# mueller-franzes/medfusion

Measured on AMD Instinct MI355X. Metric: images/sec at 256x256, 150 DDIM steps (DiffusionPipeline.sample incl. VAE decode), higher is better.
Workload: dtype f32 (emulated: fp16 pairs -- 23-bit operands, and 23-bit STORAGE of the tensors between the UNet's conv blocks: they exist as fp16 pairs only)

## Files before the change

### medfusion_amd/csrc/conv_f16x2.h

```cpp
#pragma once
#include "common.h"
#include "split_f16.h"

#ifndef MFC2_HZ
#define MFC2_HZ 0
#endif
#ifndef MFC2_OUT_STORE
#define MFC2_OUT_STORE 0
#endif

namespace mfc2 {
using namespace mf;

typedef float f32x16 __attribute__((ext_vector_type(16)));
typedef float f32x4 __attribute__((ext_vector_type(4)));
typedef unsigned int u32x4 __attribute__((ext_vector_type(4)));
typedef _Float16 f16x8 __attribute__((ext_vector_type(8)));
typedef _Float16 f16x2 __attribute__((ext_vector_type(2)));

struct FuseP {
  int on, act;
  float eps, bconst;
  double count;
  const float* gamma;
  const float* beta;
  const float* res_f32;
  const void* res_pairs;
  const float* res_bound;
  const float* res_slots;
  int res_nslots;
  int tiles_per_sample;
  const float* emb;
  long emb_stride;
  const float* emb_bound;
  float* out_f32;
  void* out_pairs;
  float* out_bound;
  unsigned* rv;
  unsigned* rv_err;
};

struct ConvP2 {
  const void* x1;
  const void* x2;
  const void* w;
  const float* bias;
  float* y;
  const float* bound1;
  const float* bound2;
  int wexp;
  float* out_bound;
  int bound_slots;
  int N, Hin, Win, C1, C2, Cin, Cout;
  int Hout, Wout, Heff, Weff, KH, KW, stride, pad;
  int M, K, HWout;
  int cgroups, cg_per_split, splitk;
  int tiles_m, tiles_n;
  long slab;
  unsigned bytes1, bytes2, bytesw;
  int subpix, hw_src;
  int out_nt;
  int wphase_rows;
  int walk_n_fast;
  double* gn_partial;
  int gn_groups, gn_parts, gn_cpg;
  int tree;
  float* handoff;
  unsigned* sync;
  FuseP fz;
  void* y_pairs;
  float* y_pair_bound;
  float wl1_1, wl1_2, bmax;
#if MFC2_HZ & (256 | 512)
  float* dbg;
#endif
};

__device__ __forceinline__ int xcd_remap2(int bid, int total) {
  const int q = total >> 3, r = total & 7;
  const int xcd = bid & 7, within = bid >> 3;
  const int base = xcd < r ? xcd * (q + 1) : r * (q + 1) + (xcd - r) * q;
  return base + within;
}

#ifndef MFC2_HZ
#define MFC2_HZ 0
#endif
#define MFC2_HZ_ON(BIT) ((MFC2_HZ >> (BIT)) & 1)
#ifndef MFC2_HZ_PAD
#define MFC2_HZ_PAD 7
#endif

__device__ __forceinline__ float hz_add(float a, float b) { float r; asm volatile("v_add_f32 %0, %1, %2" : "=v"(r) : "v"(a), "v"(b)); return r; }
__device__ __forceinline__ float hz_mul(float a, float b) { float r; asm volatile("v_mul_f32 %0, %1, %2" : "=v"(r) : "v"(a), "v"(b)); return r; }

#define MFC2_WAIT_VM(N) asm volatile("s_waitcnt vmcnt(%0)" ::"n"(N) : "memory")
#if MFC2_HZ & 512
#define MFC2_STAMP(I) { if (p.dbg && threadIdx.x == 0) reinterpret_cast<unsigned long*>(p.dbg)[(long)MFC2_BID * 8 + (I)] = __builtin_amdgcn_s_memrealtime(); }
#else
#define MFC2_STAMP(I)
#endif
#define MFC2_WAIT_LGKM0() asm volatile("s_waitcnt lgkmcnt(0)" ::: "memory")

#define MFC2_BODY_AS_KERNEL 1
#define MFC2_BID blockIdx.x
#include "conv_f16x2_body.inc"
#undef MFC2_BODY_AS_KERNEL
#undef MFC2_BID
#define MFC2_BODY_AS_KERNEL 0
#define MFC2_BID bid
#include "conv_f16x2_body.inc"
#undef MFC2_BODY_AS_KERNEL
#undef MFC2_BID

__global__ __launch_bounds__(256) void split_act_f16x2_kernel(const float* __restrict__ x, u32x4* __restrict__ out, long octets,
                                                              const float* __restrict__ bound, long octets_per_row) {
  const long stride = (long)gridDim.x * blockDim.x;
  for (long o = (long)blockIdx.x * blockDim.x + threadIdx.x; o < octets; o += stride) {
    const float sc = bound ? exp2i(-scale_exp_of(bound[o / octets_per_row])) : 1.f;
    const f32x4 v0 = *reinterpret_cast<const f32x4*>(x + o * 8) * sc, v1 = *reinterpret_cast<const f32x4*>(x + o * 8 + 4) * sc;
    u32x4 hi, lo;
    split8_f16(v0, v1, hi, lo);
    out[o * 2] = hi;
    out[o * 2 + 1] = lo;
  }
}

__global__ __launch_bounds__(256) void split_act_slots_kernel(const float* __restrict__ x, u32x4* __restrict__ out, long octets_per_row,
                                                              const float* __restrict__ slots, int nslots, float* __restrict__ bound_out) {
  __shared__ float sm[4];
  const int row = blockIdx.y, tid = threadIdx.x;
  float m = 0.f;
  for (int i = tid; i < nslots; i += 256) m = fmaxf(m, slots[(long)row * nslots + i]);
  m = mf::wave_max(m);
  if ((tid & 63) == 0) sm[tid >> 6] = m;
  __syncthreads();
  const float b = fmaxf(fmaxf(sm[0], sm[1]), fmaxf(sm[2], sm[3]));
  if (blockIdx.x == 0 && tid == 0) bound_out[row] = b;
  const float sc = exp2i(-scale_exp_of(b));
  const long base = (long)row * octets_per_row;
  for (long o = (long)blockIdx.x * 256 + tid; o < octets_per_row; o += (long)gridDim.x * 256) {
    const f32x4 v0 = *reinterpret_cast<const f32x4*>(x + (base + o) * 8) * sc, v1 = *reinterpret_cast<const f32x4*>(x + (base + o) * 8 + 4) * sc;
    u32x4 hi, lo;
    split8_f16(v0, v1, hi, lo);
    out[(base + o) * 2] = hi;
    out[(base + o) * 2 + 1] = lo;
  }
}

}
```

### medfusion_amd/csrc/conv_f16x2.hip

```cpp
#include "common.h"
#include <string.h>
#include <mutex>
#include <vector>
#include "gn_partial.h"
#include "conv_plan.h"
#include "conv_f16x2.h"
#include "conv_f16x2_halo.h"
#include "conv_f16x2_group.h"
#include "winograd.h"

using namespace mf;

namespace {

struct Tile2 { int id, BM, BN, WM, WN, NST, HG; };
const Tile2 kTiles2[] = {
    {31, 128, 256, 2, 4, 3, 0}, {32, 256, 128, 4, 2, 3, 0}, {33, 128, 128, 2, 4, 3, 0}, {34, 128, 128, 4, 2, 3, 0}, {35, 256, 64, 4, 2, 3, 0},
    {36, 128, 64, 4, 2, 3, 0}, {37, 64, 256, 1, 8, 3, 0},
    {51, 128, 128, 2, 2, 2, 0}, {52, 128, 128, 2, 2, 3, 0}, {53, 64, 128, 2, 2, 3, 0}, {54, 128, 64, 2, 2, 3, 0},
    {61, 256, 128, 4, 2, 3, 6}, {62, 256, 128, 4, 2, 3, 7}, {63, 128, 128, 2, 4, 3, 4}, {64, 128, 128, 2, 4, 3, 5},
};
inline size_t tile_lds(const Tile2& t) {
  return t.HG ? (size_t)2 * t.HG * (t.WM * t.WN) * 1024 + (size_t)3 * t.BN * 128 : (size_t)t.NST * (t.BM + t.BN) * 128;
}
// ... 338 lines not shown
  return igemm_plan_query(d, tile_id, splitk);
}

int mf_split_f16x2(const float* x, void* xs, const float* bound, int rows, int64_t per_row, void* stream) {
  MF_REQUIRE(x && xs && rows > 0 && per_row > 0 && per_row % 8 == 0, MF_EINVAL, "split_f16x2: bad args (per_row %% 8 == 0)");
  const long octets = (long)rows * (per_row / 8);
  ProfScope ps(MF_FAM_MISC, (hipStream_t)stream, 0, 8.0 * rows * (double)per_row);
  const int blocks = (int)((octets + 255) / 256 > 8192 ? 8192 : (octets + 255) / 256);
  MF_LAUNCH(mfc2::split_act_f16x2_kernel, dim3(blocks), dim3(256), 0, (hipStream_t)stream, x, reinterpret_cast<mfc2::u32x4*>(xs), octets, bound,
                     (long)(per_row / 8));
  return check_launch("split_f16x2");
}

int mf_split_f16x2_slots(const float* x, void* xs, const float* slots, int nslots, float* bound_out, int rows, int64_t per_row, void* stream) {
  MF_REQUIRE(x && xs && slots && bound_out && nslots > 0 && rows > 0 && rows <= 65535 && per_row > 0 && per_row % 8 == 0, MF_EINVAL,
             "split_f16x2_slots: bad args (per_row %% 8 == 0, rows <= 65535)");
  const long opr = per_row / 8;
  ProfScope ps(MF_FAM_MISC, (hipStream_t)stream, 0, 8.0 * rows * (double)per_row);
  long bpr = (opr + 255) / 256;
  const long cap = (8192 + rows - 1) / rows;
  if (bpr > cap) bpr = cap;
  MF_LAUNCH(mfc2::split_act_slots_kernel, dim3((int)bpr, rows), dim3(256), 0, (hipStream_t)stream, x, reinterpret_cast<mfc2::u32x4*>(xs), opr, slots, nslots,
            bound_out);
  return check_launch("split_f16x2_slots");
}

static int host_scale_exp(float bound) {
  if (!(bound > 0.f)) return 0;
  uint32_t u;
  memcpy(&u, &bound, 4);
  const int s = (int)((u >> 23) & 0xffu) - 127 - 14;
  return s < -100 ? -100 : (s > 100 ? 100 : s);
}

int mf_conv2d_plan_override(const MfConvDesc* d, int tile, int splitk) {
  MF_REQUIRE(d && pair_precision(d->precision), MF_EINVAL, "plan_override: a MF_CONV_FP32_F16X2 / MF_CONV_F16 descriptor");
  std::lock_guard<std::mutex> lk(g_plan_mu);
  const int Cin = d->C1 + d->C2;
  for (size_t i = 0; i < g_plan_overrides.size(); ++i) {
    const PlanEntry& e = g_plan_overrides[i];
    if (e.N == d->N && e.H == d->Hin && e.W == d->Win && e.Cin == Cin && e.Cout == d->Cout && e.k == d->KH && e.stride == d->stride && e.ups == d->upsample) {
      g_plan_overrides.erase(g_plan_overrides.begin() + i);
      break;
    }
  }
  if (tile > 0 && splitk > 0) g_plan_overrides.push_back(PlanEntry{d->N, d->Hin, d->Win, Cin, d->Cout, d->KH, d->stride, d->upsample, tile, splitk});
  return MF_OK;
}

int mf_conv2d_f16x2_sync_words(const MfConvDesc* d) {
  Plan2 pl;
  if (!d || !pair_precision(d->precision) || make_plan2(d, &pl) != MF_OK || !pl.ok || !tree_possible(d, pl)) return 0;
  return cdiv(pl.M, pl.t.BM) * (d->Cout / pl.t.BN) * (pl.splitk - 1);
}

static int fuse_tiles_per_sample(const MfConvDesc* d, const Plan2& pl, int G) {
  if (!pl.ok || G <= 0 || G > 256 || d->Cout % G || d->upsample != 0) return 0;
  if (pl.splitk > 1 && !tree_possible(d, pl)) return 0;
  if (!epilogue_stats_ok(d, pl, G)) return 0;
  const int HW = pl.Hout * pl.Wout;
  if (HW < pl.t.BM && pl.t.BM / HW > 8) return 0;
  const long grid = (long)cdiv(pl.M, pl.t.BM) * (d->Cout / pl.t.BN) * pl.splitk;
  mfc2::ConvP2 dummy{};
  const int resident = dispatch_tile(pl.t.id, dummy, nullptr, d->precision == MF_CONV_F16 ? 1 : 3, 1);
  if (resident <= 0 || grid > resident) return 0;
  static const int fault = [] { const char* e = getenv("MEDFUSION_FUSE_FAULT"); return e ? atoi(e) : 0; }();
  return (HW >= pl.t.BM ? HW / pl.t.BM : 1) * (d->Cout / pl.t.BN) + (fault ? 1 : 0);
}

int mf_conv2d_f16x2_fuse_words(const MfConvDesc* d, int G) {
  Plan2 pl;
  if (!d || !pair_precision(d->precision) || make_plan2(d, &pl) != MF_OK || !pl.ok) return 0;
  return fuse_tiles_per_sample(d, pl, G) > 0 ? 2 * d->N : 0;
}

struct PairsOut { void* y_split; float* y_bound; float wl1_1, wl1_2, bmax; };
static int conv_f16x2_impl(const void* x1s, const void* x2s, const void* ws, const float* bias, float* y, const float* x1_bound, const float* x2_bound,
                           float w_bound, float* y_bound, void* workspace, size_t workspace_bytes, uint32_t* sync, double* gn_partial, int G,
                           const MfGnFuse* fz, const MfConvDesc* d, void* stream, const PairsOut* po = nullptr);

int mf_conv2d_f16x2_pairs_out_ok(const MfConvDesc* d) {
  Plan2 pl;
  if (!d || !pair_precision(d->precision) || make_plan2(d, &pl) != MF_OK || !pl.ok || d->Cout % 8) return 0;
  return (pl.splitk == 1 || tree_possible(d, pl)) ? 1 : 0;
}

int mf_conv2d_f16x2_pairs_out(const void* x1s, const void* x2s, const void* ws, const float* bias, float* y, void* y_split, float* y_bound_out,
                              const float* x1_bound, const float* x2_bound, float w_bound, float w_l1_1, float w_l1_2, float bias_max, void* workspace,
                              size_t workspace_bytes, uint32_t* sync, const MfConvDesc* d, void* stream) {
  MF_REQUIRE(y && y_split && y_bound_out && x1_bound, MF_EINVAL, "conv(f16x2, pairs out): y, y_split, y_bound_out and x1_bound are required");
  MF_REQUIRE(d && (d->C2 == 0 || x2_bound), MF_EINVAL, "conv(f16x2, pairs out): x2_bound with a second source");
  MF_REQUIRE(mf_conv2d_f16x2_pairs_out_ok(d), MF_EUNSUPPORTED, "conv(f16x2, pairs out): this plan reduces split-K behind the launch (mf_conv2d_f16x2_pairs_out_ok == 0)");
  MF_REQUIRE(w_l1_1 >= 0.f && w_l1_2 >= 0.f && bias_max >= 0.f, MF_EINVAL, "conv(f16x2, pairs out): norms must be >= 0");
  const PairsOut po{y_split, y_bound_out, w_l1_1, w_l1_2, bias_max};
  return conv_f16x2_impl(x1s, x2s, ws, bias, y, x1_bound, x2_bound, w_bound, nullptr, workspace, workspace_bytes, sync, nullptr, 0, nullptr, d, stream, &po);
}

int mf_conv2d_f16x2(const void* x1s, const void* x2s, const void* ws, const float* bias, float* y, const float* x1_bound, const float* x2_bound,
                    float w_bound, float* y_bound, void* workspace, size_t workspace_bytes, uint32_t* sync, double* gn_partial, int G,
                    const MfConvDesc* d, void* stream) {
  MF_REQUIRE(y, MF_EINVAL, "conv(f16x2): null pointer");
  return conv_f16x2_impl(x1s, x2s, ws, bias, y, x1_bound, x2_bound, w_bound, y_bound, workspace, workspace_bytes, sync, gn_partial, G, nullptr, d, stream);
}

int mf_conv2d_f16x2_gn_apply(const void* x1s, const void* x2s, const void* ws, const float* bias, const float* x1_bound, const float* x2_bound,
                             float w_bound, void* workspace, size_t workspace_bytes, uint32_t* sync, double* gn_partial, int G, const MfGnFuse* f,
                             const MfConvDesc* d, void* stream) {
  MF_REQUIRE(f && gn_partial && G > 0, MF_EINVAL, "conv_gn_apply: needs the fuse arguments, the record array and G");
  MF_REQUIRE(f->out_split && f->out_bound && f->rendezvous && f->error_flag, MF_EINVAL, "conv_gn_apply: out_split, out_bound, rendezvous and error_flag are required");
  MF_REQUIRE((f->gamma == nullptr) == (f->beta == nullptr), MF_EINVAL, "conv_gn_apply: gamma/beta must both be given or both NULL");
  MF_REQUIRE(!(f->residual && f->residual_pairs), MF_EINVAL, "conv_gn_apply: the residual is fp32 OR fp16 pairs");
  MF_REQUIRE(!f->residual_pairs || f->res_bound, MF_EINVAL, "conv_gn_apply: a residual given as fp16 pairs needs the res_bound that scaled it");
  MF_REQUIRE(!f->residual || f->res_bound || (f->res_bound_slots && f->res_nslots > 0), MF_EINVAL, "conv_gn_apply: a residual needs res_bound or res_bound_slots");
  MF_REQUIRE(!f->emb || (f->emb_bound && f->emb_stride % 4 == 0), MF_EINVAL, "conv_gn_apply: an embedding needs emb_bound and emb_stride %% 4 == 0");
  return conv_f16x2_impl(x1s, x2s, ws, bias, nullptr, x1_bound, x2_bound, w_bound, nullptr, workspace, workspace_bytes, sync, gn_partial, G, f, d, stream);
}

struct Prep { mfc2::ConvP2 p; Plan2 pl; bool tree; double flops, bytes; int terms; };
static int conv_f16x2_prepare(const void* x1s, const void* x2s, const void* ws, const float* bias, float* y, const float* x1_bound, const float* x2_bound,
                              float w_bound, float* y_bound, void* workspace, size_t workspace_bytes, uint32_t* sync, double* gn_partial, int G,
                              const MfGnFuse* fz, const MfConvDesc* d, const PairsOut* po, Prep* out, bool wino_gemm = false) {
  MF_REQUIRE(d && pair_precision(d->precision), MF_EINVAL, "conv(f16x2): desc.precision must be MF_CONV_FP32_F16X2 (or the opt-in MF_CONV_F16)");
  MF_REQUIRE((d->upsample == 3) == wino_gemm, MF_EINVAL, "conv(f16x2): upsample = 3 is internal to mf_conv2d_wino_f16x2");
  Plan2& pl = out->pl;
  mfc2::ConvP2& p = out->p;
  int rc = make_plan2(d, &pl);
  if (rc) return rc;
  MF_REQUIRE(pl.ok, MF_EUNSUPPORTED, "conv(f16x2): this shape/layout is not on the fp16-pair path (ask mf_conv2d_f16x2_ok)");
  MF_REQUIRE(x1s && ws && (y || fz), MF_EINVAL, "conv(f16x2): null pointer");
  MF_REQUIRE(d->C2 == 0 || x2s != nullptr, MF_EINVAL, "conv(f16x2): C2 > 0 but x2 is null");
  MF_REQUIRE(!gn_partial || gn_parts2(d, pl, G) > 0, MF_EUNSUPPORTED, "conv(f16x2): cannot emit GroupNorm partials (mf_conv2d_gn_parts == 0)");
  MF_REQUIRE(!y_bound || (!gn_partial && bound_slots2(d, pl, false) > 0), MF_EUNSUPPORTED,
             "conv(f16x2): cannot measure the output bound of this plan (mf_conv2d_f16x2_bound_slots == 0, or GroupNorm statistics requested)");
  p.x1 = x1s; p.x2 = x2s; p.w = ws; p.bias = bias; p.y = y;
  p.bound1 = x1_bound; p.bound2 = x2_bound; p.wexp = host_scale_exp(w_bound); p.out_bound = y_bound; p.bound_slots = y_bound ? bound_slots2(d, pl, false) : 0;
  p.N = d->N; p.Hin = d->Hin; p.Win = d->Win; p.C1 = d->C1; p.C2 = d->C2; p.Cin = d->C1 + d->C2; p.Cout = d->Cout;
  p.Hout = pl.Hout; p.Wout = pl.Wout; p.Heff = pl.Heff; p.Weff = pl.Weff;
  p.KH = d->KH; p.KW = d->KW; p.stride = d->stride; p.pad = d->pad;
  p.subpix = d->upsample == 2 ? 1 : 0; p.hw_src = d->Hin * d->Win;
  if (p.subpix) { p.KH = p.KW = 2; p.Heff = d->Hin; p.Weff = d->Win; }
  p.M = pl.M; p.K = pl.K; p.HWout = pl.Hout * pl.Wout;
  p.cgroups = pl.cgroups; p.cg_per_split = pl.cg_per_split; p.splitk = pl.splitk;
  p.tiles_m = cdiv(pl.M, pl.t.BM); p.tiles_n = d->Cout / pl.t.BN;
  p.slab = (long)pl.M * d->Cout;
  p.bytes1 = (unsigned)(4.0 * d->N * d->Hin * d->Win * d->C1);
  p.bytes2 = (unsigned)(4.0 * d->N * d->Hin * d->Win * d->C2);
  p.bytesw = (unsigned)(4.0 * d->Cout * pl.K * (p.subpix ? 4 : wino_gemm ? 16 : 1));
  p.wphase_rows = wino_gemm ? (d->N / 16) * d->Hin * d->Win : 0;
  {
    static const int walk = [] { const char* e = getenv("MF_CONV_WALK"); return e ? atoi(e) : 1; }();
    const double act_bytes = 4.0 * d->N * d->Hin * d->Win * (d->C1 + d->C2), w_bytes = 4.0 * d->Cout * pl.K * (p.subpix ? 4 : 1);
    p.walk_n_fast = (!wino_gemm && p.tiles_n > 1 && (walk == 2 || (walk == 1 && act_bytes > w_bytes))) ? 1 : 0;
  }
  p.out_nt = 0;
  p.gn_partial = nullptr; p.gn_groups = G; p.gn_cpg = G > 0 ? d->Cout / G : 8; p.gn_parts = 0;
  p.tree = 0; p.handoff = nullptr; p.sync = nullptr;
#if MFC2_HZ & (256 | 512)
  p.dbg = g_conv_dbg;
#endif
  p.y_pairs = po ? po->y_split : nullptr; p.y_pair_bound = po ? po->y_bound : nullptr;
  p.wl1_1 = po ? po->wl1_1 : 0.f; p.wl1_2 = po ? po->wl1_2 : 0.f; p.bmax = po ? po->bmax : 0.f;
  memset(&p.fz, 0, sizeof(p.fz));
  if (fz) {
    const int tps = fuse_tiles_per_sample(d, pl, G);
    MF_REQUIRE(tps > 0, MF_EUNSUPPORTED, "conv_gn_apply: this plan cannot apply its GroupNorm inside the launch (mf_conv2d_f16x2_fuse_words == 0)");
    p.fz.on = 1; p.fz.act = fz->act; p.fz.eps = fz->eps; p.fz.bconst = fz->bconst; p.fz.count = (double)(pl.Hout * pl.Wout) * (d->Cout / G);
    p.fz.gamma = fz->gamma; p.fz.beta = fz->beta; p.fz.res_f32 = fz->residual; p.fz.res_pairs = fz->residual_pairs;
    p.fz.res_bound = fz->res_bound; p.fz.res_slots = fz->res_bound ? nullptr : fz->res_bound_slots; p.fz.res_nslots = fz->res_nslots;
    p.fz.tiles_per_sample = tps; p.fz.emb = fz->emb; p.fz.emb_stride = (long)fz->emb_stride; p.fz.emb_bound = fz->emb_bound;
    p.fz.out_f32 = fz->out; p.fz.out_pairs = fz->out_split; p.fz.out_bound = fz->out_bound; p.fz.rv = fz->rendezvous; p.fz.rv_err = fz->error_flag;
  }
  const bool tree = pl.splitk > 1 && tree_possible(d, pl) && (!gn_partial || epilogue_stats_ok(d, pl, G));
  if ((pl.splitk == 1 || tree) && gn_partial) { p.gn_partial = gn_partial; p.gn_parts = p.HWout >= pl.t.BM ? p.HWout / pl.t.BM : 1; }
  if (tree) {
    const size_t need = tree_handoff_bytes(d, pl);
    MF_REQUIRE(workspace && workspace_bytes >= need, MF_EWORKSPACE, "conv(f16x2): workspace %zu < %zu", workspace_bytes, need);
    MF_REQUIRE(sync, MF_EINVAL, "conv(f16x2): this plan meets its split-K slices inside the launch and needs `sync` "
                                "(mf_conv2d_f16x2_sync_words(d) zero-initialised words the caller keeps between launches)");
    p.tree = tree_mode(); p.handoff = reinterpret_cast<float*>(workspace); p.sync = sync;
    if (y_bound && p.bound_slots == 0) p.out_bound = nullptr;
  } else if (pl.splitk > 1) {
    const size_t need = (size_t)pl.splitk * pl.M * d->Cout * sizeof(float);
    MF_REQUIRE(workspace && workspace_bytes >= need, MF_EWORKSPACE, "conv(f16x2): workspace %zu < %zu", workspace_bytes, need);
    p.y = reinterpret_cast<float*>(workspace);
    p.out_bound = nullptr;
  }
  out->tree = tree;
  out->flops = 2.0 * pl.M * (double)d->Cout * (d->upsample == 2 ? 9.0 * (d->C1 + d->C2) : (double)pl.K);
  out->bytes = 4.0 * ((double)d->N * d->Hin * d->Win * p.Cin + (double)d->Cout * pl.K + (double)pl.M * d->Cout);
  out->terms = d->precision == MF_CONV_F16 ? 1 : 3;
  return MF_OK;
}

static int conv_f16x2_impl(const void* x1s, const void* x2s, const void* ws, const float* bias, float* y, const float* x1_bound, const float* x2_bound,
                           float w_bound, float* y_bound, void* workspace, size_t workspace_bytes, uint32_t* sync, double* gn_partial, int G,
                           const MfGnFuse* fz, const MfConvDesc* d, void* stream, const PairsOut* po) {
  Prep q;
  int rc = conv_f16x2_prepare(x1s, x2s, ws, bias, y, x1_bound, x2_bound, w_bound, y_bound, workspace, workspace_bytes, sync, gn_partial, G, fz, d, po, &q);
  if (rc) return rc;
  hipStream_t s = (hipStream_t)stream;
  const Plan2& pl = q.pl;
  const mfc2::ConvP2& p = q.p;
  const bool tree = q.tree;
  {
    const int terms = q.terms;
    ProfScope ps(fz ? MF_FAM_CONV_GN_FUSED : MF_FAM_CONV_IGEMM, s, q.flops, q.bytes, 2.0 * pl.M * (double)d->Cout * pl.K * terms);
    ps.set_tag(pl.t.id + (terms == 1 ? 100000 : 0));
    rc = dispatch_tile(pl.t.id, p, s, terms, 0);
    if (rc == -1) { set_error("conv(f16x2): no tile config %d", pl.t.id); rc = MF_EINVAL; }
  }
  if (rc) return rc;
  if (pl.splitk > 1 && !tree) {
    const int HW = p.HWout;
    ProfScope ps(MF_FAM_SPLITK_REDUCE, s, 0, 4.0 * pl.M * d->Cout * (pl.splitk + 1));
    if (gn_partial) {
      const int slices = stats_slices(d->N, HW, d->Cout, G), chunks = stats_chunks(HW);
      MF_LAUNCH(gn_partial_kernel<true>, dim3(chunks, d->N, slices), dim3(kStatsThreads), stats_lds_bytes(d->Cout / slices), s,
                         reinterpret_cast<const float*>(workspace), gn_partial, HW, d->Cout, G, pl.splitk, p.slab, bias, y, (float*)nullptr);
      return check_launch("splitk_reduce_stats");
    }
    const long p4 = (long)HW * d->Cout / 4;
    int bx = (int)((p4 + 255) / 256);
    const int cap = cdiv(2048, d->N);
    if (bx > cap) bx = cap;
    MF_LAUNCH(splitk_reduce_kernel<0>, dim3(bx, d->N), dim3(256), 0, s, reinterpret_cast<const float*>(workspace), bias, y, p4, d->Cout,
                       pl.splitk, p.slab, y_bound);
    return check_launch("splitk_reduce");
  }
  return MF_OK;
}

static bool single_launch(const MfConvDesc* d, const Plan2& pl, int G) {
  if (pl.splitk == 1) return G == 0 || gn_parts2(d, pl, G) > 0;
  return tree_possible(d, pl) && (G == 0 || epilogue_stats_ok(d, pl, G));
}

int mf_conv2d_f16x2_group_ok(const MfConvDesc* a, int Ga, const MfConvDesc* b, int Gb) {
  static const int off = [] { const char* e = getenv("MF_CONV_GROUP"); return e && atoi(e) == 0 ? 1 : 0; }();
  if (off || !a || !b || a->precision != MF_CONV_FP32_F16X2 || b->precision != MF_CONV_FP32_F16X2) return 0;
  Plan2 pa, pb;
  if (make_plan2(a, &pa) != MF_OK || make_plan2(b, &pb) != MF_OK || !pa.ok || !pb.ok) return 0;
  if (!single_launch(a, pa, Ga) || !single_launch(b, pb, Gb)) return 0;
  mfc2::ConvP2 dummy{};
  return dispatch_group(pa.t.id, pb.t.id, dummy, dummy, nullptr, 2) == 1 ? 1 : 0;
}

int mf_conv2d_f16x2_group(const MfConvF16x2Call* a, const MfConvF16x2Call* b, void* stream) {
  MF_REQUIRE(a && b && a->d && b->d && a->y && b->y, MF_EINVAL, "conv_group: two calls with descriptors and outputs");
  const int Ga = a->gn_partial ? a->G : 0, Gb = b->gn_partial ? b->G : 0;
  MF_REQUIRE(mf_conv2d_f16x2_group_ok(a->d, Ga, b->d, Gb), MF_EUNSUPPORTED,
             "conv_group: these two plans cannot share a launch (mf_conv2d_f16x2_group_ok == 0: a reducer pass behind one of them, workgroup sizes "
             "that differ, or a tile pair that is not instantiated)");
  Prep qa, qb;
  int rc = conv_f16x2_prepare(a->x1s, a->x2s, a->ws, a->bias, a->y, a->x1_bound, a->x2_bound, a->w_bound, a->y_bound, a->workspace, a->workspace_bytes,
                              a->sync, a->gn_partial, a->G, nullptr, a->d, nullptr, &qa);
  if (rc) return rc;
  rc = conv_f16x2_prepare(b->x1s, b->x2s, b->ws, b->bias, b->y, b->x1_bound, b->x2_bound, b->w_bound, b->y_bound, b->workspace, b->workspace_bytes,
                          b->sync, b->gn_partial, b->G, nullptr, b->d, nullptr, &qb);
  if (rc) return rc;
  MF_REQUIRE((qa.pl.splitk == 1 || qa.tree) && (qb.pl.splitk == 1 || qb.tree), MF_EUNSUPPORTED, "conv_group: a plan needs its reducer pass");
  if (qa.tree && qb.tree) {
    const char *wa = (const char*)a->workspace, *wb = (const char*)b->workspace;
    const size_t na = tree_handoff_bytes(a->d, qa.pl), nb = tree_handoff_bytes(b->d, qb.pl);
    MF_REQUIRE(wa + na <= wb || wb + nb <= wa, MF_EINVAL, "conv_group: the two workspaces overlap");
    const uint32_t *sa = a->sync, *sb = b->sync;
    const long ca = mf_conv2d_f16x2_sync_words(a->d), cb = mf_conv2d_f16x2_sync_words(b->d);
    MF_REQUIRE(sa + ca <= sb || sb + cb <= sa, MF_EINVAL, "conv_group: the two sync arrays overlap");
  }
  MF_REQUIRE(a->y != b->y, MF_EINVAL, "conv_group: one output for two convolutions");
  hipStream_t s = (hipStream_t)stream;
  ProfScope ps(MF_FAM_CONV_IGEMM, s, qa.flops + qb.flops, qa.bytes + qb.bytes,
               2.0 * 3.0 * (qa.pl.M * (double)a->d->Cout * qa.pl.K + qb.pl.M * (double)b->d->Cout * qb.pl.K));
  ps.set_tag(1000 + 100 * qa.pl.t.id + qb.pl.t.id);
  rc = dispatch_group(qa.pl.t.id, qb.pl.t.id, qa.p, qb.p, s, 0);
  if (rc == -1) { set_error("conv_group: no tile pair (%d, %d)", qa.pl.t.id, qb.pl.t.id); rc = MF_EINVAL; }
  return rc;
}

int mf_prof_tag_name(int family, int tag, char* buf, int n) {
  MF_REQUIRE(buf && n > 0, MF_EINVAL, "mf_prof_tag_name: bad args");
  auto tile_of = [](int id) -> const Tile2* { for (const auto& k : kTiles2) if (k.id == id) return &k; return nullptr; };
  auto tile_type = [&](int id, char* o, int m) {
    const Tile2* t = tile_of(id);
    if (!t) { snprintf(o, m, "?"); return; }
    if (t->HG) snprintf(o, m, "mfc2::HaloTile<%d, %d, %d, %d, %d>", t->BM, t->BN, t->WM, t->WN, t->HG);
    else snprintf(o, m, "mfc2::PlainTile<%d, %d, %d, %d, %d>", t->BM, t->BN, t->WM, t->WN, t->NST);
  };
  if ((family == MF_FAM_CONV_IGEMM || family == MF_FAM_CONV_GN_FUSED) && tag > 0) {
    const int terms = tag >= 100000 ? 1 : 3, id = tag % 100000;
    if (id >= 1000) {
      char a[96], b[96];
      tile_type((id - 1000) / 100, a, sizeof a);
      tile_type((id - 1000) % 100, b, sizeof b);
      snprintf(buf, n, "void mfc2::conv_group_kernel<%s, %s, 3>(mfc2::ConvP2, mfc2::ConvP2, int)", a, b);
      return MF_OK;
    }
    if (const Tile2* t = tile_of(id)) {
      if (t->HG) snprintf(buf, n, "void mfc2::conv_halo_kernel<%d, %d, %d, %d, %d, %d>(mfc2::ConvP2)", t->BM, t->BN, t->WM, t->WN, t->HG, terms);
      else snprintf(buf, n, "void mfc2::conv_f16x2_kernel<%d, %d, %d, %d, %d, %d>(mfc2::ConvP2)", t->BM, t->BN, t->WM, t->WN, t->NST, terms);
      return MF_OK;
    }
  }
  snprintf(buf, n, "%s (tag %d)", mf_prof_family_name(family), tag);
  return MF_OK;
}

// ... 4 lines not shown
```

### medfusion_amd/csrc/conv_f16x2_body.inc

```
template <int BM, int BN, int WM, int WN, int NST, int TERMS = 3>
#if MFC2_BODY_AS_KERNEL
__global__ __launch_bounds__(WM * WN * 64, 2) void conv_f16x2_kernel(const ConvP2 p) {
#else
__device__ __forceinline__ void conv_f16x2_body(const ConvP2& p, const int bid) {
#endif
  static_assert(TERMS == 3 || TERMS == 1, "three product terms (fp16 pairs) or one (fp16)");
  constexpr int PC = TERMS == 3 ? 2 : 1;
  constexpr int NW = WM * WN;
  static_assert(NW == 8 || NW == 4, "4 or 8 waves");
  constexpr int FM = BM / WM, FN = BN / WN, TM = FM / 32, TN = FN / 32;
  static_assert(TM >= 1 && TN >= 1 && FM % 32 == 0 && FN % 32 == 0, "per-wave footprint");
  constexpr int GP = BM / (8 * NW), GQ = BN / (8 * NW), NL = GP + GQ;
  static_assert(BM % (8 * NW) == 0 && BN % (8 * NW) == 0, "tile");
  constexpr int ROWB = 128, STAGE = (BM + BN) * ROWB;
  constexpr int NM = TERMS * TM * TN;
  constexpr int NR = PC * (TM + TN);
  constexpr int NF = (2 * NM + 2) / 3;
  static_assert(NST >= 2 && NST <= 6 && NST * STAGE <= 160 * 1024 && (NST - 1) * NL <= 63, "LDS stages");
  static_assert((NR + NF - 1) / NF <= 3, "at most three reads per slot");

  extern __shared__ __attribute__((aligned(1024))) char smem[];
  MFC2_STAMP(0)

  const int tid = threadIdx.x, lane = tid & 63;
  const int wave = __builtin_amdgcn_readfirstlane(tid >> 6);
  const int wm = wave / WN, wn = wave % WN;

  const int total = p.tiles_m * p.tiles_n * p.splitk;
  const int logical = xcd_remap2(MFC2_BID, total);
  int tile_m = logical % p.tiles_m;
  const int rest = logical / p.tiles_m;
  int tile_n = rest % p.tiles_n;
  int kz = rest / p.tiles_n;
  if (p.walk_n_fast) {
    tile_n = logical % p.tiles_n;
    const int r1 = logical / p.tiles_n;
    tile_m = r1 % p.tiles_m;
    kz = r1 / p.tiles_m;
  }
  if (p.wphase_rows) {
    const int tpc = p.wphase_rows / BM, ncomp = p.tiles_m / tpc;
    const int tm_in = logical % tpc, r1 = logical / tpc;
    tile_n = r1 % p.tiles_n;
    const int r2 = r1 / p.tiles_n;
    tile_m = (r2 % ncomp) * tpc + tm_in;
    kz = r2 / ncomp;
  }
  const int m0 = tile_m * BM, n0 = tile_n * BN;
  const int cg_beg = kz * p.cg_per_split;
  const int cg_end = min(p.cgroups, cg_beg + p.cg_per_split);
  const int taps = p.KH * p.KW;
  const int nit = (cg_end - cg_beg) * taps;

  const int lrow = lane >> 3;
  const unsigned slot16 = (unsigned)(((lane & 7) ^ ((4 * (wave & 1) + (lane >> 4)) & 7)) * 16);
  int a_pix[GP], a_inv[GP];
  const bool small_m = p.M < (1 << 23);
  const float r_hw = 1.0f / (float)p.HWout, r_w = 1.0f / (float)(p.subpix ? p.Win : p.Wout), r_src = 1.0f / (float)p.hw_src;
  auto qdiv = [small_m](int a, int d, float rd) {
    if (!small_m) return a / d;
    int q = (int)((float)a * rd);
    const int r = a - q * d;
    q += (r >= d ? 1 : 0) - (r < 0 ? 1 : 0);
    return q;
  };
#pragma unroll
  for (int i = 0; i < GP; ++i) {
    const int m = m0 + 8 * (wave + NW * i) + lrow;
    int n_ = 0, iy0 = -(1 << 28), ix0 = 0;
    if (m < p.M) {
      const int n = qdiv(m, p.HWout, r_hw);
      const int rem = m - n * p.HWout;
      n_ = n * p.Hin;
      if (p.subpix) {
        const int ph = qdiv(rem, p.hw_src, r_src), r2 = rem - ph * p.hw_src;
        const int y = qdiv(r2, p.Win, r_w), x = r2 - y * p.Win;
        iy0 = y + (ph >> 1) - 1;
        ix0 = x + (ph & 1) - 1;
      } else {
        const int oy = qdiv(rem, p.Wout, r_w), ox = rem - oy * p.Wout;
        iy0 = oy * p.stride - p.pad;
        ix0 = ox * p.stride - p.pad;
      }
    }
    unsigned vy = 0, vx = 0;
#pragma unroll
    for (int t = 0; t < 3; ++t) {
      vy |= (t < p.KH && (unsigned)(iy0 + t) < (unsigned)p.Heff ? 1u : 0u) << t;
      vx |= (t < p.KW && (unsigned)(ix0 + t) < (unsigned)p.Weff ? 1u : 0u) << t;
    }
    const unsigned valid = ((vy & 1u) ? vx : 0u) | ((vy & 2u) ? vx << p.KW : 0u) | ((vy & 4u) ? vx << (2 * p.KW) : 0u);
    a_inv[i] = (int)~valid;
    a_pix[i] = (n_ + iy0) * p.Win + ix0;
  }
  const __amdgpu_buffer_rsrc_t rsw = __builtin_amdgcn_make_buffer_rsrc(const_cast<void*>(p.w), 0, p.bytesw, 0x00020000);
  const int phase_t = p.subpix ? ((m0 % p.HWout) / p.hw_src) : (p.wphase_rows ? m0 / p.wphase_rows : 0);
  const unsigned kbytes = (unsigned)p.K * 4u;
  const unsigned qv = (unsigned)(phase_t * p.Cout + n0 + 8 * wave + lrow) * kbytes + slot16;

  int l_cc = cg_beg, l_ky = 0, l_kx = 0, l_it = 0, l_st = 0;
  unsigned pbase[GP], l_off[GP];
  unsigned l_cs4 = 0, l_so = 0;
  int l_lds = 0;
  __amdgpu_buffer_rsrc_t l_rs = rsw;

#define MFC2_CHUNK_SETUP()                                                                                              \
  {                                                                                                                     \
    const int c0_ = l_cc * 32;                                                                                          \
    const bool first_ = c0_ < p.C1;                                                                                     \
    l_cs4 = (unsigned)(first_ ? p.C1 : p.C2) * 4u;                                                                      \
    const unsigned cb4_ = (unsigned)(first_ ? c0_ : c0_ - p.C1) * 4u + slot16;                                          \
    l_rs = __builtin_amdgcn_make_buffer_rsrc(const_cast<void*>(first_ ? p.x1 : p.x2), 0, first_ ? p.bytes1 : p.bytes2, 0x00020000); \
    _Pragma("unroll") for (int i = 0; i < GP; ++i) pbase[i] = (unsigned)a_pix[i] * l_cs4 + cb4_;                        \
  }
#define MFC2_LOAD_PREP()                                                                                                \
  {                                                                                                                     \
    const unsigned ts_ = (unsigned)(l_ky * p.KW + l_kx);                                                                \
    const unsigned tapb_ = (unsigned)(l_ky * p.Win + l_kx) * l_cs4;                                                     \
    _Pragma("unroll") for (int i = 0; i < GP; ++i) l_off[i] = (pbase[i] + tapb_) | (unsigned)__builtin_amdgcn_sbfe(a_inv[i], ts_, 1u); \
    l_so = (ts_ * (unsigned)p.Cin + (unsigned)l_cc * 32u) * 4u;                                                         \
    l_lds = l_st * STAGE + wave * 1024;                                                                                 \
  }
#define MFC2_LOAD_UNIT(U)                                                                                               \
  {                                                                                                                     \
    constexpr int u_ = (U);                                                                                             \
    if constexpr (u_ < GP) {                                                                                            \
      const unsigned off_ = l_off[u_];    \
      __builtin_amdgcn_raw_ptr_buffer_load_lds(l_rs, (__attribute__((address_space(3))) void*)(smem + l_lds + NW * u_ * 1024), 16, off_, 0, 0, 0); \
    } else {                                                                                                            \
      constexpr int q_ = u_ - GP;                                                                                       \
      __builtin_amdgcn_raw_ptr_buffer_load_lds(rsw, (__attribute__((address_space(3))) void*)(smem + l_lds + BM * ROWB + NW * q_ * 1024), 16, qv, \
                                               l_so + (unsigned)q_ * (8u * NW) * kbytes, 0, 0);                         \
    }                                                                                                                   \
  }
#define MFC2_LOAD_ADVANCE()                  \
  {                                          \
    ++l_it;                                  \
    l_st = l_st == NST - 1 ? 0 : l_st + 1;   \
    ++l_kx;                                  \
    if (l_kx == p.KW) { l_kx = 0; ++l_ky; }  \
    if (l_ky == p.KH) {                      \
      l_ky = 0;                              \
      ++l_cc;                                \
      if (l_it < nit) MFC2_CHUNK_SETUP()     \
    }                                        \
  }
#define MFC2_LOAD_ALL()                                            \
  {                                                                \
    MFC2_LOAD_PREP()                                               \
    MFC2_LOAD_UNIT(0) MFC2_LOAD_UNIT(1)                            \
    if constexpr (NL > 2) MFC2_LOAD_UNIT(NL > 2 ? 2 : 0)           \
    if constexpr (NL > 3) MFC2_LOAD_UNIT(NL > 3 ? 3 : 0)           \
    if constexpr (NL > 4) MFC2_LOAD_UNIT(NL > 4 ? 4 : 0)           \
    if constexpr (NL > 5) MFC2_LOAD_UNIT(NL > 5 ? 5 : 0)           \
    if constexpr (NL > 6) MFC2_LOAD_UNIT(NL > 6 ? 6 : 0)           \
    if constexpr (NL > 7) MFC2_LOAD_UNIT(NL > 7 ? 7 : 0)           \
  }

  const int fkey = (lane >> 1) & 7, fh = lane >> 5;
  int foff[2][2];
#pragma unroll
  for (int s = 0; s < 2; ++s)
#pragma unroll
    for (int c = 0; c < 2; ++c) foff[s][c] = (lane & 31) * ROWB + (((4 * s + 2 * fh + c) ^ fkey) * 16);
  const int xrow0 = wm * FM * ROWB;
  const int wrow0 = BM * ROWB + wn * FN * ROWB;

  f32x16 accm[TM][TN], accx[TM][TN];
#pragma unroll
  for (int i = 0; i < TM; ++i)
#pragma unroll
    for (int j = 0; j < TN; ++j)
#pragma unroll
      for (int r = 0; r < 16; ++r) { accm[i][j][r] = 0.f; accx[i][j][r] = 0.f; }

  f16x8 fx[2][TM][2], fw[2][TN][2];

  const bool first_src1 = cg_beg * 32 < p.C1, last_src2 = (cg_end - 1) * 32 >= p.C1;
  const int it_sw = __builtin_amdgcn_readfirstlane((first_src1 && last_src2) ? (p.C1 / 32 - cg_beg) * taps : -1);
#ifndef MFC2_EXPS_EARLY
#define MFC2_EXPS_EARLY 1
#endif
#if MFC2_EXPS_EARLY
#define MFC2_PIXEL_EXPS_DECL()                                                                                          \
  float pb1[TM] = {}, pb2[TM] = {};    \
  f32x4 eb0 = {0.f, 0.f, 0.f, 0.f}, eb1 = {0.f, 0.f, 0.f, 0.f};
#define MFC2_PIXEL_EXPS_LOAD()                                                                                          \
  _Pragma("unroll") for (int i = 0; i < TM; ++i) {                                                                      \
    const int pm_ = min(m0 + wm * FM + i * 32 + (lane & 31), p.M - 1);                                                  \
    const int pn_ = pm_ / p.HWout;                                                                                      \
    pb1[i] = p.bound1 ? p.bound1[pn_] : 0.f;                                                                            \
    pb2[i] = (p.bound2 && p.C2 > 0) ? p.bound2[pn_] : 0.f;                                                              \
  }                                                                                                                     \
  if ((p.splitk == 1 || p.tree) && p.bias) {                                                                            \
    const int bc0_ = n0 + wn * FN + (lane % (FN / 8)) * 8;                                                              \
    eb0 = *reinterpret_cast<const f32x4*>(p.bias + bc0_);                                                               \
    eb1 = *reinterpret_cast<const f32x4*>(p.bias + bc0_ + 4);                                                           \
  }
#define MFC2_PIXEL_EXPS(I) const int e1_ = p.bound1 ? scale_exp_of(pb1[I]) : 0, e2_ = (p.bound2 && p.C2 > 0) ? scale_exp_of(pb2[I]) : 0;
#else
#define MFC2_PIXEL_EXPS_DECL()
#define MFC2_PIXEL_EXPS_LOAD()
#define MFC2_PIXEL_EXPS(I)                                                                                              \
    const int pm_ = min(m0 + wm * FM + (I) * 32 + (lane & 31), p.M - 1);                                                \
    const int pn_ = pm_ / p.HWout;                                                                                      \
    const int e1_ = p.bound1 ? scale_exp_of(p.bound1[pn_]) : 0;                                                         \
    const int e2_ = (p.bound2 && p.C2 > 0) ? scale_exp_of(p.bound2[pn_]) : 0;
#endif
  MFC2_PIXEL_EXPS_DECL()
#define MFC2_SOURCE_SWITCH()                                                                                            \
  if (__builtin_expect(it == it_sw, 0)) {                                                                               \
    if constexpr (MFC2_HZ_ON(0)) asm volatile("s_nop 15\n\ts_nop 15" ::: "memory");                                     \
    _Pragma("unroll") for (int i = 0; i < TM; ++i) {                                                                    \
      MFC2_PIXEL_EXPS(i)                                                                                                \
      const float f_ = exp2i(e1_) * exp2i(-e2_);                                                                        \
      _Pragma("unroll") for (int j = 0; j < TN; ++j)                                                                    \
        _Pragma("unroll") for (int r = 0; r < 16; ++r) { accm[i][j][r] *= f_; accx[i][j][r] *= f_; }                    \
    }                                                                                                                   \
  }

#define MFC2_READ_UNIT(S, SB, U)                                                                                        \
  {                                                                                                                     \
    constexpr int u_ = (U);                                                                                             \
    if constexpr (u_ < PC * TM) {                                                                                       \
      fx[S][u_ / PC][u_ % PC] = *reinterpret_cast<const f16x8*>(smem + (SB) + xrow0 + (u_ / PC) * 32 * ROWB + foff[S][u_ % PC]); \
    } else {                                                                                                            \
      constexpr int v_ = u_ - PC * TM;                                                                                  \
      fw[S][v_ / PC][v_ % PC] = *reinterpret_cast<const f16x8*>(smem + (SB) + wrow0 + (v_ / PC) * 32 * ROWB + foff[S][v_ % PC]); \
    }                                                                                                                   \
  }
#define MFC2_MFMA(S, N_)                                                                                                \
  {                                                                                                                     \
    constexpr int n_ = (N_);                                                                                            \
    constexpr int j_ = n_ % TN, i_ = (n_ / TN) % TM, t_ = n_ / (TN * TM);                                               \
    if constexpr (t_ == 0) accm[i_][j_] = __builtin_amdgcn_mfma_f32_32x32x16_f16(fw[S][j_][0], fx[S][i_][0], accm[i_][j_], 0, 0, 0); \
    if constexpr (t_ == 1) accx[i_][j_] = __builtin_amdgcn_mfma_f32_32x32x16_f16(fw[S][j_][0], fx[S][i_][PC - 1], accx[i_][j_], 0, 0, 0); \
    if constexpr (t_ == 2) accx[i_][j_] = __builtin_amdgcn_mfma_f32_32x32x16_f16(fw[S][j_][PC - 1], fx[S][i_][0], accx[i_][j_], 0, 0, 0); \
  }

  if (nit > 0) {
    MFC2_CHUNK_SETUP()
    MFC2_LOAD_ALL()
    MFC2_LOAD_ADVANCE()
#pragma unroll
    for (int k = 1; k < NST; ++k)
      if (nit > k) { MFC2_LOAD_ALL() MFC2_LOAD_ADVANCE() }
    MFC2_PIXEL_EXPS_LOAD()
    {
      const int g = min(nit, NST) - 1;
      if (g >= 5) { MFC2_WAIT_VM(5 * NL <= 63 ? 5 * NL : 0); } else if (g == 4) { MFC2_WAIT_VM(4 * NL <= 63 ? 4 * NL : 0); }
      else if (g == 3) { MFC2_WAIT_VM(3 * NL); } else if (g == 2) { MFC2_WAIT_VM(2 * NL); } else if (g == 1) { MFC2_WAIT_VM(NL); } else { MFC2_WAIT_VM(0); }
    }
    __builtin_amdgcn_s_barrier();
    MFC2_STAMP(1)
    MFC2_READ_UNIT(0, 0, 0) MFC2_READ_UNIT(0, 0, 1)
    if constexpr (NR > 2) MFC2_READ_UNIT(0, 0, NR > 2 ? 2 : 0)
    if constexpr (NR > 3) MFC2_READ_UNIT(0, 0, NR > 3 ? 3 : 0)
    if constexpr (NR > 4) { MFC2_READ_UNIT(0, 0, NR > 4 ? 4 : 0) MFC2_READ_UNIT(0, 0, NR > 4 ? 5 : 0) }
    if constexpr (NR > 6) { MFC2_READ_UNIT(0, 0, NR > 6 ? 6 : 0) MFC2_READ_UNIT(0, 0, NR > 6 ? 7 : 0) }
  }

#define MFC2_SLOT_A(N_, SB)                                                                                             \
  {                                                                                                                     \
    MFC2_MFMA(0, N_)                                                                                                    \
    __builtin_amdgcn_sched_barrier(0);     \
    constexpr int lo_ = (N_) < NF ? ((N_) * NR + NF - 1) / NF : NR, hi_ = (N_) < NF ? (((N_) + 1) * NR + NF - 1) / NF : NR; \
    if constexpr (lo_ < hi_ && lo_ < NR) MFC2_READ_UNIT(1, SB, lo_ < NR ? lo_ : 0)                                      \
    if constexpr (lo_ + 1 < hi_ && lo_ + 1 < NR) MFC2_READ_UNIT(1, SB, lo_ + 1 < NR ? lo_ + 1 : 0)                      \
    if constexpr (lo_ + 2 < hi_ && lo_ + 2 < NR) MFC2_READ_UNIT(1, SB, lo_ + 2 < NR ? lo_ + 2 : 0)                      \
    if constexpr ((N_) == NM - 1) MFC2_LOAD_PREP()                    \
    __builtin_amdgcn_sched_barrier(0);                                                                                  \
  }
#define MFC2_SLOT_B(N_, SB, DO_LOAD)                                                                                    \
  {                                                                                                                     \
    MFC2_MFMA(1, N_)                                                                                                    \
    __builtin_amdgcn_sched_barrier(0);                                                                                  \
    constexpr int lo_ = (N_) < NF ? ((N_) * NR + NF - 1) / NF : NR, hi_ = (N_) < NF ? (((N_) + 1) * NR + NF - 1) / NF : NR; \
    if constexpr (lo_ < hi_ && lo_ < NR) MFC2_READ_UNIT(0, SB, lo_ < NR ? lo_ : 0)                                      \
    if constexpr (lo_ + 1 < hi_ && lo_ + 1 < NR) MFC2_READ_UNIT(0, SB, lo_ + 1 < NR ? lo_ + 1 : 0)                      \
    if constexpr (lo_ + 2 < hi_ && lo_ + 2 < NR) MFC2_READ_UNIT(0, SB, lo_ + 2 < NR ? lo_ + 2 : 0)                      \
    constexpr int ll_ = ((N_) * NL + NM - 1) / NM, lh_ = (((N_) + 1) * NL + NM - 1) / NM;                               \
    if (DO_LOAD) {                                                                                                      \
      if constexpr (ll_ < lh_ && ll_ < NL) MFC2_LOAD_UNIT(ll_ < NL ? ll_ : 0)                                           \
      if constexpr (ll_ + 1 < lh_ && ll_ + 1 < NL) MFC2_LOAD_UNIT(ll_ + 1 < NL ? ll_ + 1 : 0)                           \
      if constexpr (ll_ + 2 < lh_ && ll_ + 2 < NL) MFC2_LOAD_UNIT(ll_ + 2 < NL ? ll_ + 2 : 0)                           \
      if constexpr (ll_ + 3 < lh_ && ll_ + 3 < NL) MFC2_LOAD_UNIT(ll_ + 3 < NL ? ll_ + 3 : 0)                           \
      if constexpr (ll_ + 4 < lh_ && ll_ + 4 < NL) MFC2_LOAD_UNIT(ll_ + 4 < NL ? ll_ + 4 : 0)                           \
      if constexpr (ll_ + 5 < lh_ && ll_ + 5 < NL) MFC2_LOAD_UNIT(ll_ + 5 < NL ? ll_ + 5 : 0)                           \
      if constexpr (ll_ + 6 < lh_ && ll_ + 6 < NL) MFC2_LOAD_UNIT(ll_ + 6 < NL ? ll_ + 6 : 0)                           \
      if constexpr (ll_ + 7 < lh_ && ll_ + 7 < NL) MFC2_LOAD_UNIT(ll_ + 7 < NL ? ll_ + 7 : 0)                           \
    }                                                                                                                   \
    __builtin_amdgcn_sched_barrier(0);                                                                                  \
  }
#define MFC2_REP12(M_, ...)                                                                                             \
  M_(0, __VA_ARGS__)                                                                                                    \
  if constexpr (NM > 1) { M_(NM > 1 ? 1 : 0, __VA_ARGS__) }                                                             \
  if constexpr (NM > 2) { M_(NM > 2 ? 2 : 0, __VA_ARGS__) }                                                             \
  if constexpr (NM > 3 && NM <= 4) { M_(NM > 3 ? 3 : 0, __VA_ARGS__) }                                                  \
  if constexpr (NM > 4) { M_(NM > 3 ? 3 : 0, __VA_ARGS__) M_(NM > 3 ? 4 : 0, __VA_ARGS__) M_(NM > 3 ? 5 : 0, __VA_ARGS__) } \
  if constexpr (NM > 6) { M_(NM > 6 ? 6 : 0, __VA_ARGS__) M_(NM > 6 ? 7 : 0, __VA_ARGS__) M_(NM > 6 ? 8 : 0, __VA_ARGS__)   \
                          M_(NM > 6 ? 9 : 0, __VA_ARGS__) M_(NM > 6 ? 10 : 0, __VA_ARGS__) M_(NM > 6 ? 11 : 0, __VA_ARGS__) }

  int st = 0, it = 0;
  for (; it + NST < nit; ++it) {
    MFC2_SOURCE_SWITCH()
    const int sb = st * STAGE;
    const int sn = (st == NST - 1 ? 0 : st + 1) * STAGE;
    MFC2_REP12(MFC2_SLOT_A, sb)
    MFC2_WAIT_LGKM0();
    MFC2_WAIT_VM((NST - 2) * NL);
    __builtin_amdgcn_s_barrier();
    __builtin_amdgcn_sched_barrier(0);
    MFC2_REP12(MFC2_SLOT_B, sn, true)
    MFC2_LOAD_ADVANCE()
    st = st == NST - 1 ? 0 : st + 1;
  }
  for (; it < nit; ++it) {
    MFC2_SOURCE_SWITCH()
    const int sb = st * STAGE;
    const int sn = (st == NST - 1 ? 0 : st + 1) * STAGE;
    MFC2_REP12(MFC2_SLOT_A, sb)
    MFC2_WAIT_LGKM0();
    {
      const int r = nit - 1 - it;
      if (r >= 5) { MFC2_WAIT_VM(4 * NL <= 63 ? 4 * NL : 0); } else if (r == 4) { MFC2_WAIT_VM(3 * NL); } else if (r == 3) { MFC2_WAIT_VM(2 * NL); }
      else if (r == 2) { MFC2_WAIT_VM(NL); } else { MFC2_WAIT_VM(0); }
    }
    __builtin_amdgcn_s_barrier();
    __builtin_amdgcn_sched_barrier(0);
    MFC2_REP12(MFC2_SLOT_B, sn, false)
    st = st == NST - 1 ? 0 : st + 1;
  }

  MFC2_STAMP(2)
#define MFC2_EPILOGUE_LDS_BYTES (NST * STAGE)
#include "conv_f16x2_epilogue.inc"
#undef MFC2_EPILOGUE_LDS_BYTES
  MFC2_STAMP(3)
}
```

Before: 42.52.

## Issue weight prologue loads before activation address setup in f16x2 conv

The conv kernel prologue now issues the buffer-to-LDS loads for the weight tiles of all pipeline stages first, before computing per-pixel activation addresses, so weight fetch latency overlaps the index arithmetic. The activation loads follow, and the initial vmcnt wait is adjusted to the new issue order. A constexpr checker validates that the counted waits remain correct under this order. It also adds a cheap address path for Winograd-phase GEMMs that skips the division and validity-mask computation. The default is on, with an environment variable to disable it. Risks are wait-count mistakes that would cause stale LDS reads, and extra register pressure.

Result: no change. 42.89, median of 6 (+0.9%).

```diff
diff --git a/medfusion_amd/csrc/conv_f16x2.h b/medfusion_amd/csrc/conv_f16x2.h
--- a/medfusion_amd/csrc/conv_f16x2.h
+++ b/medfusion_amd/csrc/conv_f16x2.h
@@ -61,6 +61,7 @@
   int subpix, hw_src;
   int out_nt;
   int wphase_rows;
+  int w_first;
   int walk_n_fast;
   double* gn_partial;
   int gn_groups, gn_parts, gn_cpg;
@@ -101,6 +102,30 @@
 #define MFC2_STAMP(I)
 #endif
 #define MFC2_WAIT_LGKM0() asm volatile("s_waitcnt lgkmcnt(0)" ::: "memory")
+
+constexpr bool w_first_waits_ok(int NST, int GP, int GQ, int E) {
+  const int NL = GP + GQ;
+  for (int nit = 1; nit <= 3 * NST + 2; ++nit) {
+    int last[32] = {};
+    int issued = 0, landed = 0;
+    const int np = nit < NST ? nit : NST;
+    for (int k = 0; k < np; ++k) issued += GQ;
+    for (int k = 0; k < np; ++k) { issued += GP; last[k] = issued; }
+    issued += E;
+    const int w0 = nit > 1 ? GP : 0;
+    if (issued - w0 > landed) landed = issued - w0;
+    if (landed < last[0]) return false;
+    for (int it = 0; it < nit; ++it) {
+      const bool steady = it + NST < nit;
+      const int r = nit - 1 - it;
+      const int n = steady ? (NST - 2) * NL : (r >= 5 ? (4 * NL <= 63 ? 4 * NL : 0) : (r >= 2 ? (r - 1) * NL : 0));
+      if (issued - n > landed) landed = issued - n;
+      if (it + 1 < nit && landed < last[it + 1]) return false;
+      if (steady) { issued += NL; last[it + NST] = issued; }
+    }
+  }
+  return true;
+}
 
 #define MFC2_BODY_AS_KERNEL 1
 #define MFC2_BID blockIdx.x
diff --git a/medfusion_amd/csrc/conv_f16x2.hip b/medfusion_amd/csrc/conv_f16x2.hip
--- a/medfusion_amd/csrc/conv_f16x2.hip
+++ b/medfusion_amd/csrc/conv_f16x2.hip
@@ -514,6 +514,10 @@
     const double act_bytes = 4.0 * d->N * d->Hin * d->Win * (d->C1 + d->C2), w_bytes = 4.0 * d->Cout * pl.K * (p.subpix ? 4 : 1);
     p.walk_n_fast = (!wino_gemm && p.tiles_n > 1 && (walk == 2 || (walk == 1 && act_bytes > w_bytes))) ? 1 : 0;
   }
+  {
+    static const int w_first = [] { const char* e = getenv("MF_CONV_W_FIRST"); return e ? atoi(e) : 1; }();
+    p.w_first = w_first != 0 ? 1 : 0;
+  }
   p.out_nt = 0;
   p.gn_partial = nullptr; p.gn_groups = G; p.gn_cpg = G > 0 ? d->Cout / G : 8; p.gn_parts = 0;
   p.tree = 0; p.handoff = nullptr; p.sync = nullptr;
diff --git a/medfusion_amd/csrc/conv_f16x2_body.inc b/medfusion_amd/csrc/conv_f16x2_body.inc
--- a/medfusion_amd/csrc/conv_f16x2_body.inc
+++ b/medfusion_amd/csrc/conv_f16x2_body.inc
@@ -55,44 +55,6 @@
   const int lrow = lane >> 3;
   const unsigned slot16 = (unsigned)(((lane & 7) ^ ((4 * (wave & 1) + (lane >> 4)) & 7)) * 16);
   int a_pix[GP], a_inv[GP];
-  const bool small_m = p.M < (1 << 23);
-  const float r_hw = 1.0f / (float)p.HWout, r_w = 1.0f / (float)(p.subpix ? p.Win : p.Wout), r_src = 1.0f / (float)p.hw_src;
-  auto qdiv = [small_m](int a, int d, float rd) {
-    if (!small_m) return a / d;
-    int q = (int)((float)a * rd);
-    const int r = a - q * d;
-    q += (r >= d ? 1 : 0) - (r < 0 ? 1 : 0);
-    return q;
-  };
-#pragma unroll
-  for (int i = 0; i < GP; ++i) {
-    const int m = m0 + 8 * (wave + NW * i) + lrow;
-    int n_ = 0, iy0 = -(1 << 28), ix0 = 0;
-    if (m < p.M) {
-      const int n = qdiv(m, p.HWout, r_hw);
-      const int rem = m - n * p.HWout;
-      n_ = n * p.Hin;
-      if (p.subpix) {
-        const int ph = qdiv(rem, p.hw_src, r_src), r2 = rem - ph * p.hw_src;
-        const int y = qdiv(r2, p.Win, r_w), x = r2 - y * p.Win;
-        iy0 = y + (ph >> 1) - 1;
-        ix0 = x + (ph & 1) - 1;
-      } else {
-        const int oy = qdiv(rem, p.Wout, r_w), ox = rem - oy * p.Wout;
-        iy0 = oy * p.stride - p.pad;
-        ix0 = ox * p.stride - p.pad;
-      }
-    }
-    unsigned vy = 0, vx = 0;
-#pragma unroll
-    for (int t = 0; t < 3; ++t) {
-      vy |= (t < p.KH && (unsigned)(iy0 + t) < (unsigned)p.Heff ? 1u : 0u) << t;
-      vx |= (t < p.KW && (unsigned)(ix0 + t) < (unsigned)p.Weff ? 1u : 0u) << t;
-    }
-    const unsigned valid = ((vy & 1u) ? vx : 0u) | ((vy & 2u) ? vx << p.KW : 0u) | ((vy & 4u) ? vx << (2 * p.KW) : 0u);
-    a_inv[i] = (int)~valid;
-    a_pix[i] = (n_ + iy0) * p.Win + ix0;
-  }
   const __amdgpu_buffer_rsrc_t rsw = __builtin_amdgcn_make_buffer_rsrc(const_cast<void*>(p.w), 0, p.bytesw, 0x00020000);
   const int phase_t = p.subpix ? ((m0 % p.HWout) / p.hw_src) : (p.wphase_rows ? m0 / p.wphase_rows : 0);
   const unsigned kbytes = (unsigned)p.K * 4u;
@@ -132,6 +94,20 @@
       __builtin_amdgcn_raw_ptr_buffer_load_lds(rsw, (__attribute__((address_space(3))) void*)(smem + l_lds + BM * ROWB + NW * q_ * 1024), 16, qv, \
                                                l_so + (unsigned)q_ * (8u * NW) * kbytes, 0, 0);                         \
     }                                                                                                                   \
+  }
+#define MFC2_LOAD_A_ALL()                                          \
+  {                                                                \
+    MFC2_LOAD_UNIT(0)                                              \
+    if constexpr (GP > 1) MFC2_LOAD_UNIT(GP > 1 ? 1 : 0)           \
+    if constexpr (GP > 2) MFC2_LOAD_UNIT(GP > 2 ? 2 : 0)           \
+    if constexpr (GP > 3) MFC2_LOAD_UNIT(GP > 3 ? 3 : 0)           \
+  }
+#define MFC2_LOAD_W_ALL()                                          \
+  {                                                                \
+    MFC2_LOAD_UNIT(GP)                                             \
+    if constexpr (GQ > 1) MFC2_LOAD_UNIT(GQ > 1 ? GP + 1 : GP)     \
+    if constexpr (GQ > 2) MFC2_LOAD_UNIT(GQ > 2 ? GP + 2 : GP)     \
+    if constexpr (GQ > 3) MFC2_LOAD_UNIT(GQ > 3 ? GP + 3 : GP)     \
   }
 #define MFC2_LOAD_ADVANCE()                  \
   {                                          \
@@ -157,6 +133,70 @@
     if constexpr (NL > 7) MFC2_LOAD_UNIT(NL > 7 ? 7 : 0)           \
   }
 
+  static_assert(GP <= 4 && GQ <= 4, "MFC2_LOAD_A_ALL / MFC2_LOAD_W_ALL");
+  static_assert(w_first_waits_ok(NST, GP, GQ, 0) && w_first_waits_ok(NST, GP, GQ, 2 * TM + 2), "the counted waits under the weights-first prologue (conv_f16x2.h)");
+  const bool w_first = p.w_first != 0;
+  if (w_first && nit > 0) {
+    static_assert(NST <= 4, "a prologue chunk lies in the first channel group unless the convolution has one tap");
+    const bool one_tap = taps == 1;
+#pragma unroll
+    for (int k = 0; k < NST; ++k)
+      if (nit > k) {
+        l_so = (unsigned)__builtin_amdgcn_readfirstlane((int)(((unsigned)(one_tap ? 0 : k) * (unsigned)p.Cin + (unsigned)(cg_beg + (one_tap ? k : 0)) * 32u) * 4u));
+        l_lds = k * STAGE + wave * 1024;
+        MFC2_LOAD_W_ALL()
+      }
+    __builtin_amdgcn_sched_barrier(0);
+  }
+
+  const bool small_m = p.M < (1 << 23);
+  const float r_hw = 1.0f / (float)p.HWout, r_w = 1.0f / (float)(p.subpix ? p.Win : p.Wout), r_src = 1.0f / (float)p.hw_src;
+  auto qdiv = [small_m](int a, int d, float rd) {
+    if (!small_m) return a / d;
+    int q = (int)((float)a * rd);
+    const int r = a - q * d;
+    q += (r >= d ? 1 : 0) - (r < 0 ? 1 : 0);
+    return q;
+  };
+  if (p.wphase_rows) {
+#pragma unroll
+    for (int i = 0; i < GP; ++i) {
+      const int m = m0 + 8 * (wave + NW * i) + lrow;
+      const bool in = m < p.M;
+      a_inv[i] = in ? ~1 : ~0;
+      a_pix[i] = in ? m : (int)((unsigned)(-(1 << 28)) * (unsigned)p.Win);
+    }
+  } else {
+#pragma unroll
+    for (int i = 0; i < GP; ++i) {
+      const int m = m0 + 8 * (wave + NW * i) + lrow;
+      int n_ = 0, iy0 = -(1 << 28), ix0 = 0;
+      if (m < p.M) {
+        const int n = qdiv(m, p.HWout, r_hw);
+        const int rem = m - n * p.HWout;
+        n_ = n * p.Hin;
+        if (p.subpix) {
+          const int ph = qdiv(rem, p.hw_src, r_src), r2 = rem - ph * p.hw_src;
+          const int y = qdiv(r2, p.Win, r_w), x = r2 - y * p.Win;
+          iy0 = y + (ph >> 1) - 1;
+          ix0 = x + (ph & 1) - 1;
+        } else {
+          const int oy = qdiv(rem, p.Wout, r_w), ox = rem - oy * p.Wout;
+          iy0 = oy * p.stride - p.pad;
+          ix0 = ox * p.stride - p.pad;
+        }
+      }
+      unsigned vy = 0, vx = 0;
+#pragma unroll
+      for (int t = 0; t < 3; ++t) {
+        vy |= (t < p.KH && (unsigned)(iy0 + t) < (unsigned)p.Heff ? 1u : 0u) << t;
+        vx |= (t < p.KW && (unsigned)(ix0 + t) < (unsigned)p.Weff ? 1u : 0u) << t;
+      }
+      const unsigned valid = ((vy & 1u) ? vx : 0u) | ((vy & 2u) ? vx << p.KW : 0u) | ((vy & 4u) ? vx << (2 * p.KW) : 0u);
+      a_inv[i] = (int)~valid;
+      a_pix[i] = (n_ + iy0) * p.Win + ix0;
+    }
+  }
   const int fkey = (lane >> 1) & 7, fh = lane >> 5;
   int foff[2][2];
 #pragma unroll
@@ -239,14 +279,23 @@
   }
 
   if (nit > 0) {
-    MFC2_CHUNK_SETUP()
-    MFC2_LOAD_ALL()
-    MFC2_LOAD_ADVANCE()
-#pragma unroll
-    for (int k = 1; k < NST; ++k)
-      if (nit > k) { MFC2_LOAD_ALL() MFC2_LOAD_ADVANCE() }
-    MFC2_PIXEL_EXPS_LOAD()
-    {
+    if (w_first) {
+      MFC2_CHUNK_SETUP()
+      MFC2_LOAD_PREP() MFC2_LOAD_A_ALL()
+      MFC2_LOAD_ADVANCE()
+#pragma unroll
+      for (int k = 1; k < NST; ++k)
+        if (nit > k) { MFC2_LOAD_PREP() MFC2_LOAD_A_ALL() MFC2_LOAD_ADVANCE() }
+      MFC2_PIXEL_EXPS_LOAD()
+      if (nit > 1) { MFC2_WAIT_VM(GP); } else { MFC2_WAIT_VM(0); }
+    } else {
+      MFC2_CHUNK_SETUP()
+      MFC2_LOAD_ALL()
+      MFC2_LOAD_ADVANCE()
+#pragma unroll
+      for (int k = 1; k < NST; ++k)
+        if (nit > k) { MFC2_LOAD_ALL() MFC2_LOAD_ADVANCE() }
+      MFC2_PIXEL_EXPS_LOAD()
       const int g = min(nit, NST) - 1;
       if (g >= 5) { MFC2_WAIT_VM(5 * NL <= 63 ? 5 * NL : 0); } else if (g == 4) { MFC2_WAIT_VM(4 * NL <= 63 ? 4 * NL : 0); }
       else if (g == 3) { MFC2_WAIT_VM(3 * NL); } else if (g == 2) { MFC2_WAIT_VM(2 * NL); } else if (g == 1) { MFC2_WAIT_VM(NL); } else { MFC2_WAIT_VM(0); }
```
